# xander683/ConstructionScenePoseEstimation

Hardware: AMD Instinct MI355X
Metric: annotated frames/sec (RGB+seg+2D kpts) at 1920×1080, 1/2/4/8 MI355X (higher is better)
Workload: dtype f32

## Files before the change

constructionsceneposeestimation_amd/csrc/csg_kernels.hip:

```cpp
#include <math.h>

#include <algorithm>

#include <type_traits>

#include "csg_crops.h"
#include "csg_kernels.h"
#include "csg_raster_math.h"

namespace csg {

#ifndef CSG_ABLATION
#define CSG_ABLATION 0
#endif
#define DBG(d) (CSG_ABLATION ? (d) : 0u)

constexpr uint64_t kEmptyKey = ~0ull;

__device__ __forceinline__ uint32_t fbits(float f) { return __float_as_uint(f); }

template <int Ctrl, int RowMask, int BankMask>
__device__ __forceinline__ uint32_t dpp_add(uint32_t v) {
  return v + (uint32_t)__builtin_amdgcn_update_dpp(0, (int)v, Ctrl, RowMask, BankMask, false);
}
// ... 411 lines not shown
    const uint64_t t = __shfl_up(v, o, 64);
    if (lane >= o) v += t;
  }
  return v;
}

__global__ __launch_bounds__(64) void k_plan(const FrameDev* __restrict__ frames, uint32_t F, uint32_t def_rec,
                                             uint32_t def_bin, uint64_t rec_pool, uint64_t bin_pool, int use_hints,
                                             Slab* __restrict__ slab, uint64_t* __restrict__ need) {
  const int lane = threadIdx.x;
  uint64_t cr = 0, cb = 0;
  for (uint32_t f0 = 0; f0 < F; f0 += 64) {
    const uint32_t f = f0 + (uint32_t)lane;
    uint32_t rc = 0, bc = 0;
    if (f < F) {
      const uint32_t rh = use_hints ? frames[f].records_hint : 0u, bh = use_hints ? frames[f].bins_hint : 0u;
      rc = rh ? ((min(rh, 0x7FFFFFF0u) + 3u) & ~3u) : def_rec;
      bc = bh ? ((min(bh, 0x7FFFFFF0u) + 3u) & ~3u) : def_bin;
    }
    const uint64_t ir = wave_incl_scan64(rc, lane), ib = wave_incl_scan64(bc, lane);
    if (f < F) {
      Slab sl;
      sl.rec_base = min(cr + ir - rc, rec_pool);
      sl.bin_base = min(cb + ib - bc, bin_pool);
      sl.rec_cap = (uint32_t)min((uint64_t)rc, rec_pool - sl.rec_base);
      sl.bin_cap = (uint32_t)min((uint64_t)bc, bin_pool - sl.bin_base);
      sl.pad[0] = sl.pad[1] = 0u;
      slab[f] = sl;
    }
    cr += __shfl(ir, 63, 64);
    cb += __shfl(ib, 63, 64);
  }
  if (lane == 0) {
    need[0] = max(need[0], cr);
    need[1] = max(need[1], cb);
  }
}

__global__ __launch_bounds__(256) void k_scan(SceneDev s, BatchDev b) {
  __shared__ uint32_t wsum[kBlock / 64];
  __shared__ uint32_t carry;
  const uint32_t f = blockIdx.x;
  const uint32_t* tc = b.tile_count + (size_t)f * s.n_tiles;
  uint32_t* to = b.tile_off + (size_t)f * (s.n_tiles + 1);
  if (threadIdx.x == 0) carry = 0;
  __syncthreads();
  for (uint32_t base = 0; base < s.n_tiles; base += kBlock) {
    const uint32_t t = base + threadIdx.x;
    const uint32_t v = t < s.n_tiles ? tc[t] : 0u;
    uint32_t tot;
    const uint32_t ex = block_excl_scan(v, wsum, tot);
    const uint32_t c0 = carry;
    if (t < s.n_tiles) to[t] = c0 + ex;
    __syncthreads();
    if (threadIdx.x == 0) carry = c0 + tot;
    __syncthreads();
  }
  if (threadIdx.x == 0) {
    to[s.n_tiles] = carry;
    if (carry > b.slab[f].bin_cap) atomicOr(b.overflow, 2u);
  }
}

template <bool kBanded>
__global__ __launch_bounds__(256) void k_bin(SceneDev s, BatchDev b) {
  extern __shared__ uint32_t dyn[];
  uint32_t* hist = dyn;
  __shared__ uint32_t pre[kBinRound + 1];
  __shared__ uint32_t lrc[kBinRound];
  __shared__ uint32_t wsum[kBlock / 64];
  const uint32_t f = blockIdx.y;
  const int tid = threadIdx.x;
  const Slab sb = b.slab[f];
  const uint32_t n = min(b.rec_count[f * kCounterStride], sb.rec_cap);
  const uint32_t* rect = b.rect + sb.rec_base;
  const uint32_t* toff = b.tile_off + (size_t)f * (s.n_tiles + 1);
  uint32_t* bins = b.bins + sb.bin_base;
  const uint32_t* bo = b.bcount + ((size_t)f * gridDim.x + blockIdx.x) * s.n_tiles;
  const uint32_t* tcnt = b.tile_count + (size_t)f * s.n_tiles;
  const uint32_t band = min(s.n_tiles, kBinBand);
  for (uint32_t t0 = 0; t0 < s.n_tiles; t0 += band) {
    const uint32_t nb = min(band, s.n_tiles - t0);
    for (uint32_t t = tid; t < nb; t += kBlock)
      hist[t] = toff[t0 + t] + tcnt[t0 + t] - bo[t0 + t] - 1u;
    __syncthreads();
    for (uint32_t base = blockIdx.x * kBinRound; base < n; base += gridDim.x * kBinRound) {
      const uint32_t total = bin_round_setup<0>(rect, base, n, lrc, pre, wsum, s, [](int, uint32_t) {});
      __syncthreads();
      for (uint32_t j = tid; j < total; j += kBlock) {
        const int k = find_bin_item(pre, j);
        const uint32_t t = rect_tile(lrc[k], j - pre[k], s.tiles_x, s.rect_ys);
        if (!kBanded || t - t0 < nb) {
          const uint32_t slot = atomicSub(&hist[t - t0], 1u);
          if (slot < sb.bin_cap) bins[slot] = base + (uint32_t)k;
        }
      }
      __syncthreads();
    }
  }
}

template <bool Small>
__device__ __forceinline__ void row_span(const uint4& g0, const uint4& g1, int ox, int oy, int ly, int x0, int x1,
                                         int& xl, int& xr, bool no_exact) {
  using T = typename std::conditional<Small, int32_t, int64_t>::type;
  const int32_t RX[3] = {(int32_t)g0.x, (int32_t)g0.y, (int32_t)g0.z};
  const int32_t RY[3] = {(int32_t)g0.w, (int32_t)g1.x, (int32_t)g1.y};
  const int32_t OX = ox * 256, OY = oy * 256;
  const int32_t cy = ly * 256 + 128;
  T c0[3];
  int32_t dys[3];
  float lo = -1.0e30f, hi = 1.0e30f;
  const int ea[3] = {1, 2, 0}, eb[3] = {2, 0, 1};
#pragma unroll
  for (int e = 0; e < 3; ++e) {
    const int32_t ax = RX[ea[e]] - OX, ay = RY[ea[e]] - OY;
    const int32_t dx = RX[eb[e]] - RX[ea[e]];
    const int32_t dy = RY[eb[e]] - RY[ea[e]];
    const int bias = (dy < 0 || (dy == 0 && dx > 0)) ? 0 : -1;
    if constexpr (Small) c0[e] = __mul24(dx, cy - ay) + __mul24(dy, ax) + bias;
    else c0[e] = (int64_t)dx * (cy - ay) + (int64_t)dy * ax + bias;
    dys[e] = dy;
    const float t = (float)c0[e] * __builtin_amdgcn_rcpf((float)dy);
    hi = (dy > 0) ? fminf(hi, t) : hi;
    lo = (dy < 0) ? fmaxf(lo, t) : lo;
    hi = (dy == 0 && c0[e] < 0) ? -1.0e30f : hi;
  }
  constexpr float kEps = 1.0f / 64.0f;
  const float lc = (lo - 128.0f) * (1.0f / 256.0f), hc = (hi - 128.0f) * (1.0f / 256.0f);
  const float lcc = fminf(fmaxf(lc, (float)x0 - 1.0f), (float)x1 + 1.0f);
  const float hcc = fmaxf(fminf(hc, (float)x1 + 1.0f), (float)x0 - 1.0f);
  xl = max((int)ceilf(lcc - kEps), x0);
  xr = min((int)floorf(hcc + kEps), x1);
  const float fl = lcc - floorf(lcc), fh = hcc - floorf(hcc);
  const bool walk_l = lc > (float)x0 - 0.5f && lc < (float)x1 + 0.5f && (fl <= kEps || fl >= 1.0f - kEps);
  const bool walk_r = hc > (float)x0 - 0.5f && hc < (float)x1 + 0.5f && (fh <= kEps || fh >= 1.0f - kEps);
  if (no_exact) return;
  auto covers = [&](int lx) {
    const int32_t cx = lx * 256 + 128;
    bool in = true;
#pragma unroll
    for (int e = 0; e < 3; ++e) {
      if constexpr (Small) in &= c0[e] - __mul24(dys[e], cx) >= 0;
      else in &= c0[e] - (int64_t)dys[e] * cx >= 0;
    }
    return in;
  };
  if (walk_l) {
#pragma clang loop vectorize(disable) interleave(disable) unroll(disable)
    while (xl <= xr && !covers(xl)) ++xl;
  }
  if (walk_r) {
#pragma clang loop vectorize(disable) interleave(disable) unroll(disable)
    while (xr >= xl && !covers(xr)) --xr;
  }
}

#ifndef CSG_STAGE
#define CSG_STAGE (kRasterBlock >= 256 ? 124 : 64)
#endif
#ifndef CSG_WAVES
#define CSG_WAVES 7
#endif
#ifndef CSG_COV_STAGE
#define CSG_COV_STAGE (kRasterBlock >= 256 ? 72 : 38)
#endif
#ifndef CSG_COV_WAVES
#define CSG_COV_WAVES 7
#endif
#define CSG_RASTER_ATTR \
  __attribute__((amdgpu_waves_per_eu(kCov ? CSG_COV_WAVES : CSG_WAVES, kCov ? CSG_COV_WAVES : CSG_WAVES)))
constexpr int kStage = CSG_STAGE;
static_assert(kStage <= kRasterBlock && CSG_COV_STAGE <= kRasterBlock, "one staged record per thread");
constexpr int kRB = kRasterBlock;
constexpr int kL2Words = kRB * kTileW / 32;
constexpr int kColWords = (kTileW + 31) / 32;
template <bool kCov>
constexpr int kStageOf = kCov ? CSG_COV_STAGE : kStage;
template <int NS>
struct RecImage {
  uint4 q[kRecGroups][NS];
};

struct CovLds {
  uint32_t keys[kCovSlots];
  uint32_t mask[kCovSlots][kTilePix / 32];
  uint32_t ovf;
};

struct RasterCtx {
  const uint32_t* aquad;
  const uint32_t* acls;
  unsigned long long* zb;
  int ox, oy;
  float inv_near, inv_far;
  uint32_t dbg;
  uint32_t* ctr;
  CovLds* cov;
  int32_t* rlabel;
  uint32_t* gcov;
};

__device__ __forceinline__ void cov_mark(const RasterCtx& c, uint32_t label, int lx, int ly) {
  CovLds& t = *c.cov;
  const uint32_t h = label & (uint32_t)(kCovSlots - 1);
#pragma clang loop vectorize(disable) unroll(disable)
  for (uint32_t p = 0; p < (uint32_t)kCovSlots; ++p) {
    const uint32_t idx = (h + p) & (uint32_t)(kCovSlots - 1);
    uint32_t cur = t.keys[idx];
    if (cur == kNoAlpha) cur = atomicCAS(&t.keys[idx], kNoAlpha, label);
    if (cur == kNoAlpha || cur == label) {
      const uint32_t px = (uint32_t)(ly * kTileW + lx);
      atomicOr(&t.mask[idx][px >> 5], 1u << (px & 31u));
      return;
    }
  }
  t.ovf = 1u;
  atomicOr(&c.gcov[label], kCovUnknown);
}

__device__ __forceinline__ int cov_find(const RasterCtx& c, uint32_t label) {
  const CovLds& t = *c.cov;
  const uint32_t h = label & (uint32_t)(kCovSlots - 1);
#pragma clang loop vectorize(disable) unroll(disable)
  for (uint32_t p = 0; p < (uint32_t)kCovSlots; ++p) {
    const uint32_t idx = (h + p) & (uint32_t)(kCovSlots - 1);
    const uint32_t cur = t.keys[idx];
    if (cur == label) return (int)idx;
    if (cur == kNoAlpha) return -1;
  }
  return -1;
}


__device__ __forceinline__ float f_(uint32_t u) { return __uint_as_float(u); }

#ifndef CSG_ZB_SWIZZLE
#define CSG_ZB_SWIZZLE 1
#endif
__device__ __forceinline__ int zb_index(int lx, int ly) {
  return ly * kTileW + (CSG_ZB_SWIZZLE ? (lx ^ (ly & (kTileW - 1))) : lx);
}

template <bool kCov, int NS>
__device__ __forceinline__ void fragment(const RasterCtx& c, const RecImage<NS>& I, int k, int lx, int ly) {
  const float fx = (float)(c.ox + lx) + 0.5f, fy = (float)(c.oy + ly) + 0.5f;
  const uint4 g2 = I.q[2][k], g4 = I.q[4][k];
  const float invw = plane_at(f_(g2.z), f_(g2.w), f_(g4.z), fx, fy);
  if (!(invw >= c.inv_far && invw <= c.inv_near)) return;
  auto alpha_ok = [&]() {
    const uint4 g3 = I.q[3][k];
    const float r = rcp_ieee(invw);
    const f32x2 p0 = {f_(g3.x), f_(g3.y)}, p1 = {f_(g3.z), f_(g3.w)}, p2 = {f_(g4.x), f_(g4.y)};
    const f32x2 uv = ((p0 * fx + p1 * fy) + p2) * r;
    return alpha_pass(c.aquad, c.acls, (g2.y & 0xFFFFFFu) * kTexAlign, g4.w, (int)(g2.y >> 24), uv.x, uv.y);
  };
  const unsigned long long key = ((unsigned long long)(0xFFFFFFFFu - fbits(invw)) << 32) | g2.x;
  unsigned long long* z = &c.zb[zb_index(lx, ly)];
  if constexpr (kCov) {
    const int32_t lab = c.rlabel[k];
    const bool zwin = key < *z;
    int slot = -1;
    bool mark = false;
    if (lab >= 0) {
      slot = cov_find(c, (uint32_t)lab);
      const uint32_t px = (uint32_t)(ly * kTileW + lx);
      mark = slot < 0 || !((c.cov->mask[slot][px >> 5] >> (px & 31u)) & 1u);
    }
    if (!zwin && !mark) return;
    if (g2.y != kNoAlpha && !alpha_ok()) return;
    if (mark) {
      if (slot >= 0) {
        const uint32_t px = (uint32_t)(ly * kTileW + lx);
        atomicOr(&c.cov->mask[slot][px >> 5], 1u << (px & 31u));
      }
      else cov_mark(c, (uint32_t)lab, lx, ly);
    }
    if (zwin) atomicMin(z, key);
    return;
  }
  if (g2.y == kNoAlpha && !(DBG(c.dbg) & 512u)) {
    atomicMin(z, key);
    return;
  }
  if (!(DBG(c.dbg) & 16u) && key >= *z) {
    if (DBG(c.dbg) & 512u) atomicAdd(&c.ctr[7], 1u);
    return;
  }
  if (!(DBG(c.dbg) & 4u) && g2.y != kNoAlpha) {
    if (DBG(c.dbg) & 512u) {
      const uint64_t m = __ballot(1);
      if ((uint32_t)__lane_id() == (uint32_t)__ffsll((unsigned long long)m) - 1u) {
        atomicAdd(&c.ctr[12], 1u);
        atomicAdd(&c.ctr[13], (uint32_t)__popcll(m));
      }
    }
    const bool pass = alpha_ok();
    if (DBG(c.dbg) & 512u) atomicAdd(&c.ctr[pass ? 6 : 5], 1u);
    if (!pass) return;
  }
  atomicMin(z, key);
}

template <int NS>
__device__ __forceinline__ uint32_t stage_record_r(const Rec* recs, uint32_t r, uint32_t rec_cap, RecImage<NS>& img,
                                                   int slot, int ox, int oy, uint32_t& row0);
template <int NS>
__device__ __forceinline__ uint32_t stage_record(const Rec* recs, const uint32_t* bins, uint32_t idx, uint32_t end,
                                                 uint32_t rec_cap, RecImage<NS>& img, int slot, int ox, int oy,
                                                 uint32_t& row0) {
  const uint32_t r = (idx < end && slot < NS) ? bins[idx] : 0xFFFFFFFFu;
  return stage_record_r<NS>(recs, r, rec_cap, img, slot, ox, oy, row0);
}
template <int NS>
__device__ __forceinline__ uint32_t stage_record_r(const Rec* recs, uint32_t r, uint32_t rec_cap, RecImage<NS>& img,
                                                   int slot, int ox, int oy, uint32_t& row0) {
  row0 = 0;
  if (r >= rec_cap) return 0;
  const uint4* src = reinterpret_cast<const uint4*>(recs + r);
  uint4 q[kRecGroups];
#pragma unroll
  for (int k = 0; k < kRecGroups; ++k) q[k] = src[k];
#pragma unroll
  for (int k = 0; k < kRecGroups; ++k) img.q[k][slot] = q[k];
  const uint32_t p0 = q[1].z, p1 = q[1].w;
  int y0 = max((int)(p0 >> 16), oy), y1 = min((int)(p1 >> 16), oy + kTileH - 1);
  const int x0 = max((int)(p0 & 0xFFFFu), ox), x1 = min((int)(p1 & 0xFFFFu), ox + kTileW - 1);
  if (x0 > x1 || y0 > y1) return 0u;
  const int32_t X[3] = {(int32_t)q[0].x, (int32_t)q[0].y, (int32_t)q[0].z};
  const int32_t Y[3] = {(int32_t)q[0].w, (int32_t)q[1].x, (int32_t)q[1].y};
  const float sl = (float)(x0 * 256 + 128), sr = (float)(x1 * 256 + 128);
  float fx[3], fy[3];
#pragma unroll
  for (int k = 0; k < 3; ++k) { fx[k] = (float)X[k]; fy[k] = (float)(Y[k] - oy * 256); }
  float ylo = 1.0e30f, yhi = -1.0e30f;
#pragma unroll
  for (int k = 0; k < 3; ++k) {
    if (fx[k] >= sl && fx[k] <= sr) { ylo = fminf(ylo, fy[k]); yhi = fmaxf(yhi, fy[k]); }
    const int n = (k + 1) % 3;
    const float dxe = fx[n] - fx[k], dye = fy[n] - fy[k];
    const float r0 = __builtin_amdgcn_rcpf(dxe);
    const float rdx = fmaf(fmaf(-dxe, r0, 1.0f), r0, r0);
#pragma unroll
    for (int side = 0; side < 2; ++side) {
      const float xs = side ? sr : sl;
      if ((fx[k] - xs) * (fx[n] - xs) < 0.0f) {
        const float yc = fy[k] + (xs - fx[k]) * rdx * dye;
        ylo = fminf(ylo, yc);
        yhi = fmaxf(yhi, yc);
      }
    }
  }
  bool small = true;
#pragma unroll
  for (int k = 0; k < 3; ++k)
    small &= abs(X[k] - ox * 256) < (1 << 14) && abs(Y[k] - oy * 256) < (1 << 14);
  if (!(ylo <= yhi)) return 0u;
  const float wid = small ? 16.0f : 128.0f;
  const int r0 = (int)ceilf((ylo - 128.0f - wid) * (1.0f / 256.0f));
  const int r1 = (int)floorf((yhi - 128.0f + wid) * (1.0f / 256.0f));
  y0 = max(y0, oy + r0);
  y1 = min(y1, oy + r1);
  row0 = (uint32_t)(y0 - oy) | (small ? 0x80u : 0u);
  return y0 <= y1 ? (uint32_t)(y1 - y0 + 1) : 0u;
}

#ifndef CSG_PREFETCH_BIN
#define CSG_PREFETCH_BIN 1
#endif

template <int NS>
struct RasterLds {
  RecImage<NS> img;
  uint32_t starts1[NS];
  uint16_t before1[NS + 1];
  uint32_t crec[NS];
  uint8_t row0[NS];
  uint32_t span[kRB];
  uint32_t starts[kL2Words];
  uint16_t before[kL2Words + 1];
  uint32_t wsum[kRB / 64];
  uint32_t wsum2[kRB / 64];
};

template <bool kCov, int NS>
__device__ __forceinline__ void raster_block(const RasterCtx& c, const SceneDev& s, const BatchDev& b, RasterLds<NS>& L,
                                             uint32_t beg, uint32_t end, const uint32_t* bins, const Rec* recs,
                                             uint32_t rec_cap, uint32_t rfirst) {
  const int tid = threadIdx.x;
#if CSG_PREFETCH_BIN
  uint32_t rnext = rfirst;
#endif
  for (uint32_t base = beg; base < end; base += NS) {
    uint32_t row0;
#if CSG_PREFETCH_BIN
    const uint32_t rows = stage_record_r<NS>(recs, rnext, rec_cap, L.img, tid, c.ox, c.oy, row0);
    rnext = (tid < NS && base + NS + (uint32_t)tid < end) ? bins[base + NS + tid] : 0xFFFFFFFFu;
#else
    const uint32_t rows = stage_record(recs, bins, base + tid, end, rec_cap, L.img, tid, c.ox, c.oy, row0);
#endif
    if (tid < NS) L.row0[tid] = (uint8_t)row0;
    if constexpr (kCov) {
      if (tid < NS) {
        int32_t lab = -1;
        if (rows) {
          lab = s.inst[L.img.q[2][tid].x >> s.uid_shift].label;
          if (lab >= 0 && (uint32_t)lab >= b.n_labels) lab = -1;
        }
        c.rlabel[tid] = lab;
      }
    }
    if ((DBG(b.dbg) & 512u) && rows) {
      atomicAdd(&b.overflow[1], 1u);
      atomicAdd(&b.overflow[2], rows);
      const uint4 g1 = L.img.q[1][tid];
      if (((g1.w & 0xFFFFu) - (g1.z & 0xFFFFu)) < 4u && ((g1.w >> 16) - (g1.z >> 16)) < 4u) {
        atomicAdd(&b.overflow[9], 1u);
        atomicAdd(&b.overflow[10], rows);
      }
    }
    if (tid < NS) L.starts1[tid] = 0u;
    if (tid == 0) L.before1[0] = 0;
    uint32_t tot1p;
    const uint32_t ex1p = block_excl_scan<false, kRB>(rows | (rows ? 0x10000u : 0u), L.wsum, tot1p);
    const uint32_t tot1 = tot1p & 0xFFFFu;
    if (rows) {
      const uint32_t ex1 = ex1p & 0xFFFFu, ci = ex1p >> 16, e_end = ex1 + rows;
      L.crec[ci] = (uint32_t)tid | (ex1 << 8);
      atomicOr(&L.starts1[ex1 >> 5], 1u << (ex1 & 31u));
      if ((e_end & ~31u) > ex1) L.before1[e_end >> 5] = (uint16_t)(ci + 1u);
    }
    __syncthreads();
    for (uint32_t c1 = 0; c1 < ((DBG(b.dbg) & 256u) ? 0u : tot1); c1 += kRB) {
      const uint32_t j1 = c1 + tid;
      uint32_t w2 = 0, sp = 0;
      int xl = 0;
      if (j1 < tot1) {
        const uint32_t w1 = L.starts1[j1 >> 5], nb1 = L.before1[j1 >> 5];
        const uint32_t cr = L.crec[nb1 + (uint32_t)__popc(w1 & (0xFFFFFFFFu >> (31u - (j1 & 31u)))) - 1u];
        const int k = (int)(cr & 255u);
        const uint32_t first = cr >> 8;
        const uint4 g0 = L.img.q[0][k], g1 = L.img.q[1][k];
        const int x0 = max((int)(g1.z & 0xFFFFu) - c.ox, 0), x1 = min((int)(g1.w & 0xFFFFu) - c.ox, kTileW - 1);
        const uint32_t r0b = L.row0[k];
        const int ly = (int)(r0b & 31u) + (int)(j1 - first);
        int xr;
        if (DBG(b.dbg) & 1024u) { xl = 1; xr = 0; }
        else if (r0b & 0x80u) row_span<true>(g0, g1, c.ox, c.oy, ly, x0, x1, xl, xr, DBG(b.dbg) & 2048u);
        else {
          if (DBG(b.dbg) & 512u) atomicAdd(&b.overflow[8], 1u);
          row_span<false>(g0, g1, c.ox, c.oy, ly, x0, x1, xl, xr, DBG(b.dbg) & 2048u);
        }
        if (xl <= xr) {
          w2 = (uint32_t)(xr - xl + 1);
          sp = (uint32_t)k | ((uint32_t)ly << 8);
        }
      }
      if ((DBG(b.dbg) & 512u) && w2) {
        atomicAdd(&b.overflow[3], 1u);
        atomicAdd(&b.overflow[4], w2);
        const uint4 g1 = L.img.q[1][sp & 255u];
        if (((g1.w & 0xFFFFu) - (g1.z & 0xFFFFu)) < 4u && ((g1.w >> 16) - (g1.z >> 16)) < 4u)
          atomicAdd(&b.overflow[11], w2);
      }
      if constexpr (kL2Words >= kRB) {
#pragma unroll
        for (int w = 0; w < kL2Words / kRB; ++w) L.starts[tid + w * kRB] = 0u;
      } else if (tid < kL2Words) {
        L.starts[tid] = 0u;
      }
      if (tid == 0) L.before[0] = 0;
      uint32_t totp;
      const uint32_t exp = block_excl_scan<false, kRB>(w2 | (w2 ? 0x10000u : 0u), L.wsum2, totp);
      const uint32_t ex2 = exp & 0xFFFFu, tot2 = totp & 0xFFFFu;
      if (w2) {
        const uint32_t ci = exp >> 16, e_end = ex2 + w2;
        L.span[ci] = sp | ((ex2 - (uint32_t)xl + (uint32_t)kTileW) << 16);
        atomicOr(&L.starts[ex2 >> 5], 1u << (ex2 & 31u));
        if constexpr (kTileW <= 32) {
          if ((e_end & ~31u) > ex2) L.before[e_end >> 5] = (uint16_t)(ci + 1u);
        } else {
          for (uint32_t d = (ex2 >> 5) + 1u; d <= (e_end >> 5); ++d) L.before[d] = (uint16_t)(ci + 1u);
        }
      }
      __syncthreads();
      for (uint32_t j = tid; j < ((DBG(b.dbg) & 8u) ? 0u : tot2); j += kRB) {
        if (DBG(b.dbg) & 512u) {
          const uint64_t m = __ballot(1);
          if ((uint32_t)__lane_id() == (uint32_t)__ffsll((unsigned long long)m) - 1u) {
            atomicAdd(&b.overflow[14], 1u);
            atomicAdd(&b.overflow[15], (uint32_t)__popcll(m));
          }
        }
        const uint32_t w = L.starts[j >> 5], nb = L.before[j >> 5];
        const uint32_t rank = nb + (uint32_t)__popc(w & (0xFFFFFFFFu >> (31u - (j & 31u))));
        const uint32_t spj = L.span[rank - 1u];
        fragment<kCov>(c, L.img, (int)(spj & 255u), (int)(j + (uint32_t)kTileW - (spj >> 16)), (int)((spj >> 8) & 255u));
      }
      __syncthreads();
    }
  }
}

struct ShadeEntry {
  float P[16];
  int32_t label;
  int32_t tex;
  uint32_t base;
  uint32_t q01, q2;
  uint32_t n01, n2;
};

__device__ __forceinline__ void shade_setup(const SceneDev& s, const BatchDev& b, uint32_t f, uint32_t uid,
                                            ShadeEntry& e) {
  const uint32_t i = uid >> s.uid_shift, g = uid & ((1u << s.uid_shift) - 1u);
  const uint32_t set = b.fset[f];
  const float* tp = s.tri_pos + (size_t)g * 9;
  float p[9];
#pragma unroll
  for (int z = 0; z < 9; ++z) p[z] = tp[z];
  const InstSetDev is = b.iset[(size_t)set * s.n_inst + i];
  e.label = is.label;
  const int tex = is.tex;
  e.tex = tex;
  e.base = is.base;
  const float* tu = s.tri_uv + (size_t)g * 6;
#pragma unroll
  for (int z = 0; z < 6; ++z) e.P[10 + z] = tex >= 0 ? tu[z] : 0.0f;
  bool facing = false;
  if (tex >= 0 || b.depth || b.points || b.normals) {
    Cv3 v[3];
    const float* Cm = b.clip + ((size_t)f * s.n_inst + i) * 12;
#pragma unroll
    for (int z = 0; z < 3; ++z) {
      v[z].x = dot4(Cm + 0, p[3 * z], p[3 * z + 1], p[3 * z + 2]);
      v[z].y = dot4(Cm + 4, p[3 * z], p[3 * z + 1], p[3 * z + 2]);
      v[z].w = dot4(Cm + 8, p[3 * z], p[3 * z + 1], p[3 * z + 2]);
    }
    Hom h;
    hom_setup(v, h);
#pragma unroll
    for (int z = 0; z < 3; ++z) { e.P[z] = h.A[z]; e.P[3 + z] = h.B[z]; e.P[6 + z] = h.C[z]; }
    e.P[9] = h.invdet;
    facing = h.invdet < 0.0f;
  }
  float e1[3], e2[3];
  {
    const float* M = b.models + ((size_t)set * s.n_inst + i) * 16;
#pragma unroll
    for (int r = 0; r < 3; ++r) {
      const float w0 = dot4(M + 4 * r, p[0], p[1], p[2]);
      const float w1 = dot4(M + 4 * r, p[3], p[4], p[5]);
      const float w2 = dot4(M + 4 * r, p[6], p[7], p[8]);
      e1[r] = w1 - w0;
      e2[r] = w2 - w0;
    }
  }
  const float nx = e1[1] * e2[2] - e1[2] * e2[1];
  const float ny = e1[2] * e2[0] - e1[0] * e2[2];
  const float nz = e1[0] * e2[1] - e1[1] * e2[0];
  const float nn = (nx * nx + ny * ny) + nz * nz;
  const LightDev& L = b.lights[set];
  float cs = 0.0f;
  uint32_t n01 = 0, n2 = 0;
  if (nn > 0.0f) {
    const float len = sqrtf(nn);
    const float d = (nx * L.sun_dir[0] + ny * L.sun_dir[1]) + nz * L.sun_dir[2];
    cs = fabsf(d / len);
    if (b.normals) {
      const float sg = facing ? 1.0f : -1.0f;
      n01 = half_bits(sg * (nx / len)) | (half_bits(sg * (ny / len)) << 16);
      n2 = half_bits(sg * (nz / len));
    }
  }
  e.n01 = n01;
  e.n2 = n2;
  uint32_t q[3];
#pragma unroll
  for (int z = 0; z < 3; ++z) {
    const float shade = L.ambient[z] + L.sun[z] * cs;
    const int qq = (int)(shade * 256.0f + 0.5f);
    q[z] = (uint32_t)min(max(qq, 0), 65535);
  }
  e.q01 = q[0] | (q[1] << 16);
  e.q2 = q[2];
  __asm__ volatile("" ::: "memory");
  float P[16];
#pragma unroll
  for (int z = 0; z < 16; ++z) P[z] = e.P[z];
  float D[3], U[3], V[3];
  depth_plane(P, P + 3, P + 6, P[9], D);
  uv_planes(P, P + 3, P + 6, P[9], P + 10, U, V);
#pragma unroll
  for (int z = 0; z < 3; ++z) { e.P[z] = D[z]; e.P[4 + 2 * z] = U[z]; e.P[5 + 2 * z] = V[z]; }
}

__device__ __forceinline__ void shade_pixel(const SceneDev& s, const ShadeEntry& e, int px, int py, bool need_depth,
                                            uint32_t& rgb_out, int32_t& id_out, float& depth_out) {
  const bool textured = e.tex >= 0 && !(DBG(s.dbg) & 4096u);
  const float fx = (float)px + 0.5f, fy = (float)py + 0.5f;
  float r = INFINITY;
  if (need_depth || textured) r = rcp_ieee(plane_at(e.P[0], e.P[1], e.P[2], fx, fy));
  depth_out = need_depth ? r : INFINITY;
  id_out = e.label;
  int base[3] = {(int)(e.base & 255u), (int)((e.base >> 8) & 255u), (int)((e.base >> 16) & 255u)};
  int alb[3];
  if (textured) {
    const f32x2 p0 = {e.P[4], e.P[5]}, p1 = {e.P[6], e.P[7]}, p2 = {e.P[8], e.P[9]};
    const f32x2 uv = ((p0 * fx + p1 * fy) + p2) * r;
    int c[4];
    tex_sample(s, e.tex, uv.x, uv.y, c);
#pragma unroll
    for (int z = 0; z < 3; ++z) alb[z] = div255(__umul24((uint32_t)c[z], (uint32_t)base[z]) + 127u);
  } else {
#pragma unroll
    for (int z = 0; z < 3; ++z) alb[z] = base[z];
  }
  const int q[3] = {(int)(e.q01 & 0xFFFFu), (int)(e.q01 >> 16), (int)e.q2};
  uint32_t o = 0;
#pragma unroll
  for (int z = 0; z < 3; ++z) o |= (uint32_t)min((int)((__umul24((uint32_t)alb[z], (uint32_t)q[z]) + 128u) >> 8), 255) << (8 * z);
  rgb_out = o;
}

#ifndef CSG_VEC_OUT
#define CSG_VEC_OUT 1
#endif
#ifndef CSG_VEC_DEP_ONCE
#define CSG_VEC_DEP_ONCE 1
#endif

#ifndef CSG_SHADE_SLOTS
#define CSG_SHADE_SLOTS (kRasterBlock >= 256 ? 116 : 64)
#endif
constexpr uint32_t kShadeSlots = CSG_SHADE_SLOTS;
static_assert(kShadeSlots <= (uint32_t)kRasterBlock && kShadeSlots < 255u, "one setup thread per slot; 8-bit slot ids");
constexpr int kShadeProbes = 16;
struct ResolveLds {
  uint32_t keys[kShadeSlots];
  uint32_t more;
  ShadeEntry tab[kShadeSlots];
  uint32_t lstat[2 + kColWords][kMaxLdsLabels];
};

constexpr size_t lds_budget(int waves) {
  return kRasterBlock == 256
             ? (waves >= 8 ? 20480u : waves == 7 ? 22528u : waves == 6 ? 26700u : waves == 5 ? 32256u : 40960u)
             : ((157696u / (size_t)(waves * 4 / (kRasterBlock / 64))) & ~511u);
}
static_assert((sizeof(RasterLds<kStage>) > sizeof(ResolveLds) ? sizeof(RasterLds<kStage>) : sizeof(ResolveLds)) +
                      kTilePix * 8 <= lds_budget(CSG_WAVES),
              "k_raster LDS must allow CSG_WAVES workgroups per CU");

template <bool kCov>
struct RasterSide {
  RasterLds<kStageOf<kCov>> r;
};
template <>
struct RasterSide<true> {
  RasterLds<kStageOf<true>> r;
  CovLds cov;
  int32_t rlabel[kStageOf<true>];
};
static_assert((sizeof(RasterSide<true>) > sizeof(ResolveLds) ? sizeof(RasterSide<true>) : sizeof(ResolveLds)) +
                      kTilePix * 8 <= lds_budget(CSG_COV_WAVES),
              "k_raster<true> LDS must allow CSG_COV_WAVES workgroups per CU");

__device__ __forceinline__ int shade_slot(uint32_t* keys, uint32_t uid) {
  const uint32_t h = __umulhi(uid * 2654435761u, kShadeSlots);
#pragma clang loop vectorize(disable) unroll(disable)
  for (int p = 0; p < kShadeProbes; ++p) {
    uint32_t idx = h + (uint32_t)p;
    idx = idx >= kShadeSlots ? idx - kShadeSlots : idx;
    const uint32_t prev = atomicCAS(&keys[idx], kNoAlpha, uid);
    if (prev == kNoAlpha || prev == uid) return (int)idx;
  }
  return -1;
}

#ifndef CSG_SQ_X
#define CSG_SQ_X 2
#endif
#ifndef CSG_SQ_Y
#define CSG_SQ_Y 2
#endif
constexpr uint32_t kSqX = CSG_SQ_X, kSqY = CSG_SQ_Y;
constexpr uint32_t kSqN = kSqX * kSqY;
__device__ __forceinline__ bool swizzled_tile(uint32_t v, uint32_t tiles_x, uint32_t tiles_y, uint32_t& tile) {
  const uint32_t sqx = (tiles_x + kSqX - 1) / kSqX, sqy = (tiles_y + kSqY - 1) / kSqY;
  const uint32_t sq = (v / (8u * kSqN)) * 8u + (v & 7u), j = (v >> 3) % kSqN;
  if (sq >= sqx * sqy) return false;
  const uint32_t tx = (sq % sqx) * kSqX + (j % kSqX), ty = (sq / sqx) * kSqY + (j / kSqX);
  if (tx >= tiles_x || ty >= tiles_y) return false;
  tile = ty * tiles_x + tx;
  return true;
}

typedef int32_t v4i32 __attribute__((ext_vector_type(4)));
__device__ __forceinline__ void out_ids(int32_t* p, int4 v) {
  const v4i32 w = {v.x, v.y, v.z, v.w};
  __builtin_nontemporal_store(w, reinterpret_cast<v4i32*>(p));
}
#ifndef CSG_NT_OUT
#define CSG_NT_OUT 1
#endif
#ifndef CSG_NT_RGB
#define CSG_NT_RGB 1
#endif
typedef uint32_t v3u32 __attribute__((ext_vector_type(3)));
typedef float v4f32 __attribute__((ext_vector_type(4)));
typedef uint32_t v2u32 __attribute__((ext_vector_type(2)));
__device__ __forceinline__ void out_f4(float* p, float a, float b2, float c, float d) {
  const v4f32 w = {a, b2, c, d};
  if (CSG_NT_OUT) __builtin_nontemporal_store(w, reinterpret_cast<v4f32*>(p));
  else *reinterpret_cast<v4f32*>(p) = w;
}
__device__ __forceinline__ void out_u2(uint16_t* p, uint32_t a, uint32_t b2) {
  const v2u32 w = {a, b2};
  if (CSG_NT_OUT) __builtin_nontemporal_store(w, reinterpret_cast<v2u32*>(p));
  else *reinterpret_cast<v2u32*>(p) = w;
}
__device__ __forceinline__ void out_rgb4(uint8_t* p, uint32_t c0, uint32_t c1, uint32_t c2, uint32_t c3) {
  const v3u32 w = {c0 | (c1 << 24), (c1 >> 8) | (c2 << 16), (c2 >> 16) | (c3 << 8)};
  if (CSG_NT_RGB) __builtin_nontemporal_store(w, reinterpret_cast<v3u32*>(p));
  else *reinterpret_cast<v3u32*>(p) = w;
}

__device__ __forceinline__ void empty_tile(const SceneDev& s, const BatchDev& b, uint32_t f, uint32_t tile, int ox,
                                           int oy) {
  const int tid = threadIdx.x;
  if (b.n_kp && ((b.kp_tiles[(size_t)f * b.tile_words + (tile >> 5)] >> (tile & 31u)) & 1u)) {
    for (uint32_t k = tid; k < b.n_kp; k += kRB) {
      const size_t o = (size_t)f * b.n_kp + k;
      const uint32_t pp = b.kp_pix[o];
      const int px = (int)(pp & 0xFFFFu) - ox, py = (int)(pp >> 16) - oy;
      if (pp == 0xFFFFFFFFu || px < 0 || px >= kTileW || py < 0 || py >= kTileH) continue;
      b.kp_vis[o] = (b.kp_w[o] <= INFINITY) ? 2 : 1;
    }
  }
  const int ly = tid / (kTileW / 4), lx0 = (tid % (kTileW / 4)) * 4;
  const int py = oy + ly, px0 = ox + lx0;
  if (py >= (int)s.H) return;
  const size_t o = (size_t)f * s.W * s.H + (size_t)py * s.W + px0;
  const uint32_t sky = b.lights[b.fset[f]].sky & 0xFFFFFFu;
  const float nan = __builtin_nanf("");
  if (px0 + 3 < (int)s.W && ((o + b.px_align) & 3u) == 0) {
    if (b.inst) out_ids(b.inst + o, make_int4(-1, -1, -1, -1));
    if (b.rgb) out_rgb4(b.rgb + o * 3, sky, sky, sky, sky);
    if (b.depth) out_f4(b.depth + o, INFINITY, INFINITY, INFINITY, INFINITY);
    if (b.normals) {
      for (int w = 0; w < 3; ++w) out_u2(b.normals + o * 3 + 4 * w, 0u, 0u);
    }
    if (b.points) {
      for (int w = 0; w < 3; ++w) out_f4(b.points + o * 3 + 4 * w, nan, nan, nan, nan);
    }
  } else {
    for (int k = 0; k < 4 && px0 + k < (int)s.W; ++k) {
      if (b.inst) b.inst[o + k] = -1;
      if (b.rgb) {
        b.rgb[(o + k) * 3 + 0] = (uint8_t)(sky & 255u);
        b.rgb[(o + k) * 3 + 1] = (uint8_t)((sky >> 8) & 255u);
        b.rgb[(o + k) * 3 + 2] = (uint8_t)((sky >> 16) & 255u);
      }
      if (b.depth) b.depth[o + k] = INFINITY;
      if (b.normals) b.normals[(o + k) * 3 + 0] = b.normals[(o + k) * 3 + 1] = b.normals[(o + k) * 3 + 2] = 0;
      if (b.points) b.points[(o + k) * 3 + 0] = b.points[(o + k) * 3 + 1] = b.points[(o + k) * 3 + 2] = nan;
    }
  }
}

template <bool kCov>
__global__ __launch_bounds__(kRasterBlock) CSG_RASTER_ATTR void k_raster(SceneDev s, BatchDev b) {
  __shared__ unsigned long long zb[kTilePix];
  constexpr int NS = kStageOf<kCov>;
  __shared__ union Lds {
    RasterSide<kCov> ra;
    ResolveLds q;
  } L;
  const int tid = threadIdx.x;
  uint32_t tile;
  if (!swizzled_tile(blockIdx.x, s.tiles_x, s.tiles_y, tile)) return;
  const uint32_t f = blockIdx.y;
  const int ox = (int)(tile % s.tiles_x) * kTileW, oy = (int)(tile / s.tiles_x) * kTileH;
  const uint32_t* toff = b.tile_off + (size_t)f * (s.n_tiles + 1);
  const Slab sb = b.slab[f];
  const uint32_t beg = min(toff[tile], sb.bin_cap);
  const uint32_t end = (DBG(b.dbg) & 2u) ? beg : min(toff[tile + 1], sb.bin_cap);
  if (beg == end && !(DBG(b.dbg) & 2u)) {
    empty_tile(s, b, f, tile, ox, oy);
    return;
  }
  const uint32_t* bins = b.bins + sb.bin_base;
  const uint32_t rfirst = (CSG_PREFETCH_BIN && tid < NS && beg + (uint32_t)tid < end) ? bins[beg + tid] : 0xFFFFFFFFu;
  for (int p = tid; p < kTilePix; p += kRB) zb[p] = kEmptyKey;
  CovLds* covp = nullptr;
  int32_t* rlabel = nullptr;
  if constexpr (kCov) {
    covp = &L.ra.cov;
    rlabel = L.ra.rlabel;
    CovLds& covl = *covp;
    for (int p = tid; p < kCovSlots * (kTilePix / 32); p += kRB) (&covl.mask[0][0])[p] = 0u;
    if (tid < kCovSlots) covl.keys[tid] = kNoAlpha;
    if (tid == 0) covl.ovf = 0u;
  }
  const Rec* recs = b.recs + sb.rec_base;
  RasterCtx c{s.aquad, s.acls, zb, ox, oy, s.inv_near, s.inv_far, b.dbg, b.overflow, covp, rlabel,
              kCov ? b.covered + (size_t)f * b.n_labels : nullptr};
  __syncthreads();
  raster_block<kCov, NS>(c, s, b, L.ra.r, beg, end, bins, recs, sb.rec_cap, rfirst);
  __syncthreads();
  if constexpr (kCov) {
    const CovLds& covl = *covp;
    constexpr int kTPS = kRB / kCovSlots;
    static_assert(kTPS * 4 * 32 == kTilePix && kTPS <= 64, "4 words per thread, a slot's threads in one wave");
    const uint32_t sl = (uint32_t)tid / kTPS, w0 = ((uint32_t)tid % kTPS) * 4u;
    uint32_t n = 0;
#pragma unroll
    for (int w = 0; w < 4; ++w) n += (uint32_t)__popc(covl.mask[sl][w0 + w]);
#pragma unroll
    for (int o = 1; o < kTPS; o <<= 1) n += (uint32_t)__shfl_xor((int)n, o, 64);
    const uint32_t lab = covl.keys[sl];
    if ((tid % kTPS) == 0 && lab != kNoAlpha) {
      if (covl.ovf) atomicOr(&c.gcov[lab], kCovUnknown);
      else atomicAdd(&c.gcov[lab], n);
    }
    __syncthreads();
  }

  if (DBG(b.dbg) & 1u) {
    if (tid == 0 && zb[0] == 0ull && b.inst) b.inst[0] = 0;
    return;
  }
  if (b.n_kp && ((b.kp_tiles[(size_t)f * b.tile_words + (tile >> 5)] >> (tile & 31u)) & 1u)) {
    for (uint32_t k = tid; k < b.n_kp; k += kRB) {
      const size_t o = (size_t)f * b.n_kp + k;
      const uint32_t pp = b.kp_pix[o];
      const int px = (int)(pp & 0xFFFFu) - ox, py = (int)(pp >> 16) - oy;
      if (pp == 0xFFFFFFFFu || px < 0 || px >= kTileW || py < 0 || py >= kTileH) continue;
      const unsigned long long key = zb[zb_index(px, py)];
      const float d = key == kEmptyKey ? INFINITY : rcp_ieee(__uint_as_float(0xFFFFFFFFu - (uint32_t)(key >> 32)));
      b.kp_vis[o] = (b.kp_w[o] <= d) ? 2 : 1;
    }
    __syncthreads();
  }
  const bool want_stats = b.stats != nullptr;
  const uint32_t nl = want_stats ? min(b.n_labels, (uint32_t)kMaxLdsLabels) : 0u;
  uint32_t (*lstat)[kMaxLdsLabels] = L.q.lstat;
  for (uint32_t l = tid; l < nl; l += kRB) {
#pragma unroll
    for (int w = 0; w < 2 + kColWords; ++w) lstat[w][l] = 0;
  }
  const int ly = tid / (kTileW / 4), lx0 = (tid % (kTileW / 4)) * 4;
  const int py = oy + ly;
  const bool row_ok = py < (int)s.H;
  const int px0 = ox + lx0;
  unsigned long long* zrow = &zb[zb_index(lx0, ly) & ~3];
  const int zsw = CSG_ZB_SWIZZLE ? (ly & 3) : 0;
  auto zpix = [&](int k) -> unsigned long long& { return zrow[k ^ zsw]; };
  uint32_t pend = 0;
  uint32_t inmask = 0;
  __shared__ uint32_t drw[2][kRB / 64];
  {
    const uint32_t sky = b.lights[b.fset[f]].sky & 0xFFFFFFu;
    const unsigned long long bgword = (unsigned long long)sky | (0xFFFFFFFFull << 32);
    uint32_t kmn = 0xFFFFFFFFu, kmx = 0u;
#pragma unroll
    for (int k = 0; k < 4; ++k) {
      const bool in = row_ok && px0 + k < (int)s.W;
      inmask |= in ? 1u << k : 0u;
      const unsigned long long key = zpix(k);
      if (in && key != kEmptyKey) {
        pend |= 1u << k;
        kmn = min(kmn, (uint32_t)(key >> 32));
        kmx = max(kmx, (uint32_t)(key >> 32));
      } else {
        zpix(k) = bgword;
      }
    }
    if (b.drange) {
#pragma unroll
      for (int o = 32; o > 0; o >>= 1) {
        kmn = min(kmn, (uint32_t)__shfl_xor((int)kmn, o, 64));
        kmx = max(kmx, (uint32_t)__shfl_xor((int)kmx, o, 64));
      }
      if ((tid & 63) == 0) { drw[0][tid >> 6] = kmn; drw[1][tid >> 6] = kmx; }
    }
  }
  const size_t npx = (size_t)s.W * s.H;
  const size_t o = (size_t)f * npx + (size_t)py * s.W + px0;
  const uint32_t bgmask = inmask & ~pend;
  const bool need_depth = b.depth || b.points;
  auto round = [&](const bool first) __attribute__((always_inline)) -> bool {
    if ((uint32_t)tid < kShadeSlots) L.q.keys[tid] = kNoAlpha;
    __syncthreads();
    if (tid == 0) L.q.more = 0;
    if (first && b.drange && tid == 0) {
      uint32_t kmn = drw[0][0], kmx = drw[1][0];
#pragma unroll
      for (int w = 1; w < kRB / 64; ++w) { kmn = min(kmn, drw[0][w]); kmx = max(kmx, drw[1][w]); }
      if (kmn <= kmx) {
        const float dmin = rcp_ieee(__uint_as_float(0xFFFFFFFFu - kmn));
        const float dmax = rcp_ieee(__uint_as_float(0xFFFFFFFFu - kmx));
        if (__float_as_uint(dmin) < b.drange[f]) atomicMin(&b.drange[f], __float_as_uint(dmin));
        if (__float_as_uint(dmax) > b.drange[b.drange_F + f]) atomicMax(&b.drange[b.drange_F + f], __float_as_uint(dmax));
      }
    }
    uint32_t slots = 0xFFFFFFFFu;
    {
      uint32_t prev_uid = 0xFFFFFFFFu, prev_slot = 0xFFu;
#pragma unroll
      for (int k = 0; k < 4; ++k) {
        if ((pend >> k) & 1u) {
          const uint32_t uid = (uint32_t)zpix(k);
          uint32_t sl;
          if (uid == prev_uid) sl = prev_slot;
          else {
            const int r = shade_slot(L.q.keys, uid);
            sl = r < 0 ? 0xFFu : (uint32_t)r;
          }
          prev_uid = uid;
          prev_slot = sl;
          slots = (slots & ~(0xFFu << (8 * k))) | (sl << (8 * k));
        } else {
          prev_uid = 0xFFFFFFFFu;
        }
      }
    }
    __syncthreads();
    {
      const uint32_t u = (uint32_t)tid < kShadeSlots ? L.q.keys[tid] : kNoAlpha;
      if (u != kNoAlpha) {
        ShadeEntry& e = L.q.tab[tid];
        if (DBG(b.dbg) & 8192u) {
          e = ShadeEntry{};
          e.P[2] = 1.0f; e.tex = -1; e.label = 0;
        } else {
          shade_setup(s, b, f, u, e);
        }
      }
    }
    __syncthreads();
    if (row_ok) {
      int qx0 = px0, qy = py;
      asm volatile("" : "+v"(qx0), "+v"(qy));
      const size_t qo = (size_t)f * npx + (size_t)qy * s.W + qx0;
      int32_t run = -1;
      uint32_t cnt = 0, xmin = 0, xmax = 0;
      auto flush_run = [&]() {
        if (DBG(b.dbg) & 16384u) return;
        if (run >= 0 && (uint32_t)run < nl) {
          const uint32_t col = xmin - (uint32_t)ox;
          atomicAdd(&lstat[0][run], cnt);
          atomicOr(&lstat[2 + (kColWords > 1 ? col >> 5 : 0u)][run], (0xFu >> (3u - (xmax - xmin))) << (col & 31u));
          atomicOr(&lstat[1][run], 1u << ((uint32_t)qy - (uint32_t)oy));
        } else if (run >= 0 && b.stats && (uint32_t)run < b.n_labels) {
          uint32_t* st = b.stats + ((size_t)f * b.n_labels + (uint32_t)run) * 5;
          atomicAdd(&st[0], cnt);
          atomicMin(&st[1], xmin);
          atomicMin(&st[2], (uint32_t)qy);
          atomicMax(&st[3], xmax);
          atomicMax(&st[4], (uint32_t)qy);
        }
      };
      bool vec = false;
      if (CSG_VEC_OUT && (b.depth || b.normals || b.points) && inmask == 0xFu && ((qo + b.px_align) & 3u) == 0) {
        uint32_t done = first ? bgmask : 0u;
#pragma unroll
        for (int k = 0; k < 4; ++k) done |= ((slots >> (8 * k)) & 0xFFu) != 0xFFu ? 1u << k : 0u;
        vec = done == 0xFu;
      }
#pragma unroll
      for (int k = 0; k < 4; ++k) {
        const int px = qx0 + k;
        const uint32_t sl = (slots >> (8 * k)) & 0xFFu;
        const bool bg = first && ((bgmask >> k) & 1u);
        if (sl == 0xFFu && !bg) continue;
        float dep = INFINITY;
        uint32_t n01 = 0, n2 = 0;
        if (!bg) {
          const ShadeEntry& e = L.q.tab[sl];
          uint32_t rgb;
          int32_t id;
          shade_pixel(s, e, px, qy, need_depth && !(CSG_VEC_DEP_ONCE && vec), rgb, id, dep);
          n01 = e.n01;
          n2 = e.n2;
          zpix(k) = (unsigned long long)rgb | ((unsigned long long)(uint32_t)id << 32);
          pend &= ~(1u << k);
          if (want_stats) {
            if (id != run) {
              flush_run();
              run = id;
              cnt = 0;
              xmin = (uint32_t)px;
            }
            ++cnt;
            xmax = (uint32_t)px;
          }
        }
        if (vec) continue;
        if (b.depth) b.depth[qo + k] = dep;
        if (b.normals) {
          uint16_t* d = b.normals + (qo + k) * 3;
          d[0] = (uint16_t)(n01 & 0xFFFFu);
          d[1] = (uint16_t)(n01 >> 16);
          d[2] = (uint16_t)n2;
        }
        if (b.points) {
          float pt[3];
          if (bg) pt[0] = pt[1] = pt[2] = __builtin_nanf("");
          else unproject(b.cam + (size_t)f * kCamFloats, px, qy, dep, pt);
          float* d = b.points + (qo + k) * 3;
          d[0] = pt[0];
          d[1] = pt[1];
          d[2] = pt[2];
        }
      }
      flush_run();
      if (vec) {
        const uint32_t bgv = first ? bgmask : 0u;
        float dv[4];
#pragma unroll
        for (int k = 0; k < 4; ++k) {
          const ShadeEntry& e = L.q.tab[(bgv >> k) & 1u ? 0u : (slots >> (8 * k)) & 0xFFu];
          const float fx = (float)(qx0 + k) + 0.5f, fy = (float)qy + 0.5f;
          dv[k] = ((bgv >> k) & 1u) || !need_depth ? INFINITY : rcp_ieee(plane_at(e.P[0], e.P[1], e.P[2], fx, fy));
        }
        if (b.depth) out_f4(b.depth + qo, dv[0], dv[1], dv[2], dv[3]);
        if (b.normals) {
          uint32_t n01[4], n2[4];
#pragma unroll
          for (int k = 0; k < 4; ++k) {
            const bool bg = (bgv >> k) & 1u;
            const ShadeEntry& e = L.q.tab[bg ? 0u : (slots >> (8 * k)) & 0xFFu];
            n01[k] = bg ? 0u : e.n01;
            n2[k] = bg ? 0u : e.n2;
          }
          uint16_t* d = b.normals + qo * 3;
          out_u2(d, n01[0], n2[0] | (n01[1] << 16));
          out_u2(d + 4, (n01[1] >> 16) | (n2[1] << 16), n01[2]);
          out_u2(d + 8, n2[2] | (n01[3] << 16), (n01[3] >> 16) | (n2[3] << 16));
        }
        if (b.points) {
          float pt[12];
#pragma unroll
          for (int k = 0; k < 4; ++k) {
            if ((bgv >> k) & 1u) pt[3 * k] = pt[3 * k + 1] = pt[3 * k + 2] = __builtin_nanf("");
            else unproject(b.cam + (size_t)f * kCamFloats, qx0 + k, qy, dv[k], pt + 3 * k);
          }
          float* d = b.points + qo * 3;
          out_f4(d, pt[0], pt[1], pt[2], pt[3]);
          out_f4(d + 4, pt[4], pt[5], pt[6], pt[7]);
          out_f4(d + 8, pt[8], pt[9], pt[10], pt[11]);
        }
      }
    }
    if (pend) L.q.more = 1;
    __syncthreads();
    return L.q.more != 0;
  };
  if (round(true)) {
#pragma clang loop unroll(disable)
    while (round(false)) {
    }
  }
  if (row_ok) {
    uint32_t rgb[4];
    int32_t ids[4];
#pragma unroll
    for (int k = 0; k < 4; ++k) {
      const unsigned long long w = zpix(k);
      rgb[k] = (uint32_t)w;
      ids[k] = (int32_t)(w >> 32);
    }
    if (px0 + 3 < (int)s.W && ((o + b.px_align) & 3u) == 0) {
      if (b.inst) out_ids(b.inst + o, make_int4(ids[0], ids[1], ids[2], ids[3]));
      if (b.rgb) out_rgb4(b.rgb + o * 3, rgb[0], rgb[1], rgb[2], rgb[3]);
    } else {
      for (int k = 0; k < 4 && px0 + k < (int)s.W; ++k) {
        if (b.inst) b.inst[o + k] = ids[k];
        if (b.rgb) {
          b.rgb[(o + k) * 3 + 0] = (uint8_t)(rgb[k] & 255u);
          b.rgb[(o + k) * 3 + 1] = (uint8_t)((rgb[k] >> 8) & 255u);
          b.rgb[(o + k) * 3 + 2] = (uint8_t)((rgb[k] >> 16) & 255u);
        }
      }
    }
  }
  if (b.stats) {
    __syncthreads();
    uint32_t* st = b.stats + (size_t)f * b.n_labels * 5;
    for (uint32_t l = tid; l < nl; l += kRB) {
      const uint32_t cnt = lstat[0][l];
      if (cnt) {
        const uint32_t rm = lstat[1][l];
        uint32_t cm = lstat[2][l], cm_hi = cm, lo_w = 0, hi_w = 0;
#pragma unroll
// ... 578 lines not shown
```

Baseline: 25710.

## Prefetch raster records one batch ahead and split staging across two threads

The raster loop now loads the full record payload for the next batch into registers while the current batch is processed, instead of only prefetching the bin index. Each record's five 16-byte groups are split between two threads: one loads groups 0-2 and computes the row span, the other loads groups 3-4. The goal is to hide global-memory latency on record fetches and spread the load work. The cost is extra registers for the held record, which may lower occupancy, plus a second bin-index lookahead.

```diff
diff --git a/constructionsceneposeestimation_amd/csrc/csg_kernels.hip b/constructionsceneposeestimation_amd/csrc/csg_kernels.hip
--- a/constructionsceneposeestimation_amd/csrc/csg_kernels.hip
+++ b/constructionsceneposeestimation_amd/csrc/csg_kernels.hip
@@ -737,6 +737,8 @@
   atomicMin(z, key);
 }
 
+__device__ __forceinline__ uint32_t record_rows(const uint4& q0, const uint4& q1, int ox, int oy, uint32_t& row0);
+
 template <int NS>
 __device__ __forceinline__ uint32_t stage_record_r(const Rec* recs, uint32_t r, uint32_t rec_cap, RecImage<NS>& img,
                                                    int slot, int ox, int oy, uint32_t& row0);
@@ -758,12 +760,49 @@
   for (int k = 0; k < kRecGroups; ++k) q[k] = src[k];
 #pragma unroll
   for (int k = 0; k < kRecGroups; ++k) img.q[k][slot] = q[k];
-  const uint32_t p0 = q[1].z, p1 = q[1].w;
+  return record_rows(q[0], q[1], ox, oy, row0);
+}
+
+static_assert(kRecGroups == 5, "groups 0-2 on one thread, 3-4 on the other");
+struct RecHold {
+  uint4 a, b, c;
+};
+template <int NS>
+__device__ __forceinline__ int stage_slot(int tid) { return tid < NS ? tid : tid - NS; }
+template <int NS>
+__device__ __forceinline__ uint32_t stage_id(const uint32_t* bins, uint32_t idx, uint32_t end, int tid) {
+  return (tid < 2 * NS && idx < end) ? bins[idx] : 0xFFFFFFFFu;
+}
+template <int NS>
+__device__ __forceinline__ void stage_load(const Rec* recs, uint32_t r, uint32_t rec_cap, int tid, RecHold& h) {
+  if (r >= rec_cap) return;
+  const uint4* src = reinterpret_cast<const uint4*>(recs + r);
+  const int g = tid < NS ? 0 : 3;
+  h.a = src[g];
+  h.b = src[g + 1];
+  if (tid < NS) h.c = src[2];
+}
+template <int NS>
+__device__ __forceinline__ uint32_t stage_commit(const RecHold& h, uint32_t r, uint32_t rec_cap, RecImage<NS>& img,
+                                                 int tid, int ox, int oy, uint32_t& row0) {
+  row0 = 0;
+  if (r >= rec_cap) return 0;
+  const int g = tid < NS ? 0 : 3;
+  uint4* dst = &img.q[0][0] + g * NS + stage_slot<NS>(tid);
+  dst[0] = h.a;
+  dst[NS] = h.b;
+  if (tid >= NS) return 0;
+  dst[2 * NS] = h.c;
+  return record_rows(h.a, h.b, ox, oy, row0);
+}
+
+__device__ __forceinline__ uint32_t record_rows(const uint4& q0, const uint4& q1, int ox, int oy, uint32_t& row0) {
+  const uint32_t p0 = q1.z, p1 = q1.w;
   int y0 = max((int)(p0 >> 16), oy), y1 = min((int)(p1 >> 16), oy + kTileH - 1);
   const int x0 = max((int)(p0 & 0xFFFFu), ox), x1 = min((int)(p1 & 0xFFFFu), ox + kTileW - 1);
   if (x0 > x1 || y0 > y1) return 0u;
-  const int32_t X[3] = {(int32_t)q[0].x, (int32_t)q[0].y, (int32_t)q[0].z};
-  const int32_t Y[3] = {(int32_t)q[0].w, (int32_t)q[1].x, (int32_t)q[1].y};
+  const int32_t X[3] = {(int32_t)q0.x, (int32_t)q0.y, (int32_t)q0.z};
+  const int32_t Y[3] = {(int32_t)q0.w, (int32_t)q1.x, (int32_t)q1.y};
   const float sl = (float)(x0 * 256 + 128), sr = (float)(x1 * 256 + 128);
   float fx[3], fy[3];
 #pragma unroll
@@ -802,6 +841,12 @@
 
 #ifndef CSG_PREFETCH_BIN
 #define CSG_PREFETCH_BIN 1
+#endif
+#ifndef CSG_PREFETCH_REC
+#define CSG_PREFETCH_REC 1
+#endif
+#if CSG_PREFETCH_REC && !CSG_PREFETCH_BIN
+#error "CSG_PREFETCH_REC needs CSG_PREFETCH_BIN"
 #endif
 
 template <int NS>
@@ -823,12 +868,24 @@
                                              uint32_t beg, uint32_t end, const uint32_t* bins, const Rec* recs,
                                              uint32_t rec_cap, uint32_t rfirst) {
   const int tid = threadIdx.x;
-#if CSG_PREFETCH_BIN
+#if CSG_PREFETCH_REC
+  static_assert(2 * NS <= kRB, "two threads stage one record");
+  const uint32_t slot = (uint32_t)stage_slot<NS>(tid);
+  uint32_t rcur = rfirst;
+  RecHold held;
+  stage_load<NS>(recs, rcur, rec_cap, tid, held);
+  uint32_t rnext = stage_id<NS>(bins, beg + NS + slot, end, tid);
+#elif CSG_PREFETCH_BIN
   uint32_t rnext = rfirst;
 #endif
   for (uint32_t base = beg; base < end; base += NS) {
     uint32_t row0;
-#if CSG_PREFETCH_BIN
+#if CSG_PREFETCH_REC
+    const uint32_t rows = stage_commit<NS>(held, rcur, rec_cap, L.img, tid, c.ox, c.oy, row0);
+    rcur = rnext;
+    stage_load<NS>(recs, rcur, rec_cap, tid, held);
+    rnext = stage_id<NS>(bins, base + 2 * NS + slot, end, tid);
+#elif CSG_PREFETCH_BIN
     const uint32_t rows = stage_record_r<NS>(recs, rnext, rec_cap, L.img, tid, c.ox, c.oy, row0);
     rnext = (tid < NS && base + NS + (uint32_t)tid < end) ? bins[base + NS + tid] : 0xFFFFFFFFu;
 #else
@@ -1226,7 +1283,11 @@
     return;
   }
   const uint32_t* bins = b.bins + sb.bin_base;
+#if CSG_PREFETCH_REC
+  const uint32_t rfirst = stage_id<NS>(bins, beg + (uint32_t)stage_slot<NS>(tid), end, tid);
+#else
   const uint32_t rfirst = (CSG_PREFETCH_BIN && tid < NS && beg + (uint32_t)tid < end) ? bins[beg + tid] : 0xFFFFFFFFu;
+#endif
   for (int p = tid; p < kTilePix; p += kRB) zb[p] = kEmptyKey;
   CovLds* covp = nullptr;
   int32_t* rlabel = nullptr;
```

New measurement: 25930, median of 6. No clear change (+0.9%).
